# glennhickey/teHmm

Measured on AMD Instinct MI355X. Metric: genome positions/sec (Viterbi+posterior), 35 states x 10 tracks, higher is better.
Workload: dtype f64

## Files before the change

### tehmm_amd/csrc/tehmm_hip.hip

```cpp
#include <climits>
#include "tehmm_kernels.hip.h"
#include "tehmm_coop.hip.h"
#include "tehmm_lane.hip.h"
#include "tehmm_lane3.hip.h"
#include "tehmm_place.hip.h"
#include "tehmm_aux.hip.h"
#include "tehmm_fused.hip.h"
#include "tehmm_estep.hip.h"
#include "tehmm_wide_estep.hip.h"
#include "tehmm_wide.hip.h"
#include "tehmm_large.hip.h"
#include "tehmm_map.hip.h"
#include "tehmm_edist.hip.h"
#include "tehmm_segment.hip.h"
#include "tehmm_compare.hip.h"
#include "tehmm_tsd.hip.h"
#include "tehmm_masking.hip.h"
#include "tehmm_trackio.hip.h"
#include "tehmm_scaling.hip.h"

#include <algorithm>
#include <atomic>
#include <cmath>
#include <cstdio>
// ... 1146 lines not shown

template <int NT>
static void launch_vit_coop(tehmm_batch *b, const tehmm_model *m, const IntervalTab &iv,
                            const EmisTab &em, bool ratio, hipStream_t st) {
  constexpr int CPB = NT <= 44 ? 64 : 32;
  size_t lds = ((size_t)3 * CPB * (NT + 1) + 2 * (CPB + 1) * (NT + 2) + (size_t)m->lds_rows * NT) * sizeof(double);
  if (ratio) {
    allow_lds(k_vit_coop<NT, CPB, true>, lds);
    hipLaunchKernelGGL((k_vit_coop<NT, CPB, true>), dim3(b->n), dim3(256), lds, st, iv, em, m->N,
                       m->lt.p, m->ltT.p, m->pi.p, b->ratios.p, b->tb.p, b->last_state.p, b->vit_lp.p);
  } else {
    allow_lds(k_vit_coop<NT, CPB, false>, lds);
    hipLaunchKernelGGL((k_vit_coop<NT, CPB, false>), dim3(b->n), dim3(256), lds, st, iv, em, m->N,
                       m->lt.p, m->ltT.p, m->pi.p, (const double *)nullptr, b->tb.p, b->last_state.p,
                       b->vit_lp.p);
  }
}

template <int NT>
static void launch_fb_coop(tehmm_batch *b, const tehmm_model *m, const IntervalTab &iv,
                           const EmisTab &em_in, hipStream_t st) {
  constexpr int CPB = NT <= 44 ? 64 : 32;
  const EmisTab em = b->n > 256 ? without_lds_tables(em_in) : em_in;
  size_t lds = ((size_t)4 * CPB * (NT + 1) + 4 * CPB + 5 * NT + (size_t)em.lds_rows * NT) * sizeof(double);
  allow_lds(k_fb_coop<NT, CPB, false>, lds);
  hipLaunchKernelGGL((k_fb_coop<NT, CPB, false>), dim3(b->n), dim3(256), lds, st, iv, em, m->N, m->A.p,
                     m->lt.p, m->pi.p, (const double *)nullptr, b->post.p, b->beta.p, b->fwd_lp.p,
                     b->dead.p, (double *)nullptr, (int *)nullptr);
}

static int spec_chunk_size() {
  const char *s = std::getenv("TEHMM_SPEC_CHUNK");
  int cs = s ? std::atoi(s) : 512;
  if (cs <= 0) return 0;
  return std::max(64, (cs + 63) & ~63);
}

#define TEHMM_ESTEP_SMALL_DEFAULT 40

struct EvalKnobs {
  int spec_chunk;
  bool spec_chunk_set;
  int lane_sub;
  int lane_warmup;
  bool lane_probe;
  bool lane_vit;
  bool lane_p0;
  bool fused;
  bool device_place;
  bool soft_ties;
  int emis_split;
  int defer;
  int gain_window;
  bool rowindex_ref;
  bool wide;
  bool wide_cp;
  bool wide_vit;
  int wide_sub;
  int wide_vit_warmup;
  double wide_tol;
  bool wide_head;
  bool wide_poll;
  int estep_wide;
  bool estep_fused;
  int estep_small;
  int wide_estep_sq;
  bool wide_estep_serial;
};

static EvalKnobs read_eval_knobs() {
  auto num = [](const char *name, int unset) {
    const char *s = std::getenv(name);
    return s ? std::atoi(s) : unset;
  };
  EvalKnobs k;
  k.spec_chunk = spec_chunk_size();
  k.spec_chunk_set = std::getenv("TEHMM_SPEC_CHUNK") != nullptr;
  k.lane_sub = std::getenv("TEHMM_LANE_SUB") ? std::max(0, num("TEHMM_LANE_SUB", 0)) : -1;
  k.lane_warmup = std::getenv("TEHMM_LANE_WARMUP") ? std::max(1, num("TEHMM_LANE_WARMUP", 1)) : -1;
  k.lane_probe = num("TEHMM_LANE_PROBE", 1) != 0;
  k.lane_vit = num("TEHMM_LANE_VIT", 1) != 0;
  k.lane_p0 = num("TEHMM_LANE_P0", 1) != 0;
  k.fused = num("TEHMM_FUSED", 1) != 0;
  k.device_place = num("TEHMM_DEVICE_PLACE", 1) != 0;
  k.soft_ties = num("TEHMM_SOFT_TIES", 1) != 0;
  k.emis_split = std::getenv("TEHMM_EMIS_SPLIT") ? (num("TEHMM_EMIS_SPLIT", 0) != 0 ? 1 : 0) : -1;
  k.defer = num("TEHMM_DEFER", -1);
  k.gain_window = std::getenv("TEHMM_GAIN_WINDOW") ? std::max(0, num("TEHMM_GAIN_WINDOW", 0)) : -1;
  k.rowindex_ref = num("TEHMM_ROWINDEX_REF", 0) != 0;
  k.wide = num("TEHMM_WIDE", 1) != 0;
  k.wide_cp = num("TEHMM_WIDE_CP", 1) != 0;
  k.wide_vit = num("TEHMM_WIDE_VIT", 1) != 0;
  k.wide_sub = std::getenv("TEHMM_WIDE_SUB") ? std::max(32, (num("TEHMM_WIDE_SUB", 0) + 31) & ~31) : -1;
  k.wide_vit_warmup = std::max(0, num("TEHMM_WIDE_VIT_WARMUP", 32));
  k.wide_tol = 1e-8;
  if (const char *ts = std::getenv("TEHMM_WIDE_TOL")) k.wide_tol = std::min(1e-6, std::max(1e-13, std::atof(ts)));
  k.wide_head = num("TEHMM_WIDE_HEAD", 1) != 0;
  k.wide_poll = num("TEHMM_WIDE_POLL", 1) != 0;
  k.estep_wide = num("TEHMM_ESTEP_WIDE", 1);
  k.estep_fused = num("TEHMM_ESTEP_FUSED", 1) != 0;
  k.estep_small = num("TEHMM_ESTEP_SMALL", TEHMM_ESTEP_SMALL_DEFAULT);
  k.wide_estep_sq = num("TEHMM_WIDE_ESTEP_SQ", 0);
  k.wide_estep_serial = std::getenv("TEHMM_WIDE_ESTEP_SERIAL") != nullptr;
  return k;
}

static int spec_prepare(tehmm_batch *b, const tehmm_model *m, int CS) {
  SpecWork &sw = b->sw;
  if (sw.CS == CS && sw.N == m->N && sw.rows.p) return TEHMM_OK;
  sw.CS = CS;
  sw.N = m->N;
  sw.h_iv.clear();
  sw.h_t0.clear();
  sw.h_first.assign((size_t)b->n + 1, 0);
  for (int i = 0; i < b->n; ++i) {
    sw.h_first[i] = (int64_t)sw.h_iv.size();
    for (int64_t t0 = 0; t0 < b->h_len[i]; t0 += CS) {
      sw.h_iv.push_back(i);
      sw.h_t0.push_back(t0);
    }
  }
  sw.h_first[b->n] = (int64_t)sw.h_iv.size();
  sw.n_chunks = (int)sw.h_iv.size();
  const size_t nc = (size_t)std::max(1, sw.n_chunks);
  HIPCHK(sw.iv.upload(sw.h_iv.data(), sw.h_iv.size()));
  HIPCHK(sw.t0.upload(sw.h_t0.data(), sw.h_t0.size()));
  HIPCHK(sw.first.upload(sw.h_first.data(), sw.h_first.size()));
  HIPCHK(sw.e.alloc(nc));
  HIPCHK(sw.ok.alloc(nc));
  HIPCHK(sw.stats.alloc(16));
  HIPCHK(hipMemset(sw.stats.p, 0, 16 * sizeof(int)));
  HIPCHK(sw.scale.alloc(nc * (size_t)(CS / 32)));
  HIPCHK(sw.wstart.alloc(nc * (size_t)m->NP));
  HIPCHK(sw.gain.alloc(nc));
  HIPCHK(sw.wmin.alloc(nc));
  HIPCHK(sw.rows.alloc(nc * (size_t)(CS / TEHMM_VROW) * m->NP));
  HIPCHK(sw.ntie.alloc(nc));
  HIPCHK(sw.ties.alloc(nc * TEHMM_SPEC_MAXT));
  HIPCHK(sw.tierows.alloc(nc * TEHMM_SPEC_MAXT * (size_t)m->NP));
  HIPCHK(sw.segmin.alloc(nc * (TEHMM_SPEC_MAXT + 1)));
  HIPCHK(sw.offend.alloc(nc));
// ... 324 lines not shown

static int launch_vit_place(tehmm_batch *b, const tehmm_model *m, const IntervalTab &iv, int CS, int Wn, bool ratio,
                            hipStream_t st, int *n_work_max) {
  LaneWork &lw = b->lw;
  SpecWork &sw = b->sw;
  const LaneGeom lg = lane_geom(lw);
  hipLaunchKernelGGL(k_vit_place_chunks, dim3(std::max(1, b->n)), dim3(64), 0, st, iv, (const int64_t *)sw.first.p,
                     (const int64_t *)sw.t0.p, (const int64_t *)lw.ifirst.p, b->n, CS, lw.L, (const double *)lw.vgain.p,
                     (const double *)lw.slog32.p, Wn, (const int *)m->qok[ratio ? 1 : 0].p, kSpecMarginRel, kSpecCross ? 1 : 0, sw.e.p,
                     sw.gain.p);
  const int gb = (lw.n_groups + 255) / 256;
  hipLaunchKernelGGL(k_vit_place_count, dim3(std::max(1, gb)), dim3(256), 0, st, lg, (const int64_t *)sw.first.p,
                     (const int *)sw.e.p, CS, lw.place.p, lw.gclass.p);
  hipLaunchKernelGGL(k_vit_place_scan, dim3(1), dim3(64), 0, st, lw.place.p);
  hipLaunchKernelGGL(k_vit_place_fill, dim3(std::max(1, gb)), dim3(256), 0, st, lg, (const int64_t *)sw.first.p,
                     (const int *)sw.e.p, CS, lw.place.p, (const int *)lw.gclass.p, lw.wk_g.p, lw.wk_e.p, lw.wk_items.p);
  *n_work_max = 2 * lw.n_groups + TEHMM_PLACE_NE;
  return TEHMM_OK;
}

template <int NT>
static void launch_vit_stitch(tehmm_batch *b, const tehmm_model *m, const IntervalTab &iv, const VitChunks &vc,
                              hipStream_t st) {
  LaneWork &lw = b->lw;
  hipLaunchKernelGGL((k_vit_stitch<NT>), dim3((vc.n + 3) / 4), dim3(256), 0, st, iv, lane_geom(lw), vc,
                     lane_vit_items(lw), m->N, lw.soft_ties);
  hipLaunchKernelGGL((k_vit_links<NT>), dim3((vc.n + 3) / 4), dim3(256), 0, st, iv, lane_geom(lw), vc,
                     lane_vit_items(lw), m->N);
  hipLaunchKernelGGL(k_vit_runs, dim3(std::max(1, b->n)), dim3(64), 0, st, vc, b->n);
}

static LaneGeom lane_geom(const LaneWork &lw) {
  LaneGeom lg;
  lg.item_iv = lw.item_iv.p; lg.item_t0 = lw.item_t0.p; lg.ifirst = lw.ifirst.p;
  lg.n_items = lw.n_items; lg.n_groups = lw.n_groups; lg.L = lw.L;
  return lg;
}

template <int NT>
static void launch_emis_lane(tehmm_batch *b, const tehmm_model *m, const IntervalTab &iv, const EmisTab &em,
                             bool want_log, bool want_lin, bool want_f32, hipStream_t st) {
  LaneWork &lw = b->lw;
  const size_t lds = (size_t)em.lds_rows * NT * sizeof(double);
  allow_lds(k_emis_lane<NT>, lds);
  hipLaunchKernelGGL((k_emis_lane<NT>), dim3((lw.n_groups + 3) / 4), dim3(256), lds, st, iv, em, lane_geom(lw),
                     m->N, want_log ? lw.B.p : (double *)nullptr, want_lin ? lw.BH.p : (double *)nullptr, lw.MS.p,
                     want_f32 ? lw.B32.p : (float *)nullptr);
}

static bool emis_gain_split(int NT, int n_groups, int emis_split) {
  return NT >= 12 && (emis_split >= 0 ? emis_split != 0 : n_groups < 2048);
}

template <int NT>
static void launch_emis_gain_lane(tehmm_batch *b, const tehmm_model *m, const IntervalTab &iv, const EmisTab &em,
                                  int CS, int Wu, int Wn, bool ratio, int emis_split, hipStream_t st) {
  LaneWork &lw = b->lw;
  if constexpr (NT >= 12) {
    if (emis_gain_split(NT, lw.n_groups, emis_split)) {
      constexpr int NW = TEHMM_P2_NW, NU = 2;
      const size_t lds3 = Emis3Geom<NT, NW, NU>::lds_bytes(em.lds_rows);
      const dim3 grid3((lw.n_groups + NU - 1) / NU);
      if constexpr (NT <= TEHMM_RATIO_LANE_MAX) if (ratio) {
        allow_lds(k_emis_gain_lane3<NT, NW, NU, true>, lds3);
        hipLaunchKernelGGL((k_emis_gain_lane3<NT, NW, NU, true>), grid3, dim3(64 * NW * NU), lds3, st, iv, em, lane_geom(lw),
                           m->N, CS, Wu, (const float *)m->ltP.p, lw.B.p, lw.vgain.p, (const double *)b->ratios.p);
        return;
      }
      allow_lds(k_emis_gain_lane3<NT, NW, NU, false>, lds3);
      hipLaunchKernelGGL((k_emis_gain_lane3<NT, NW, NU, false>), grid3, dim3(64 * NW * NU), lds3, st, iv, em, lane_geom(lw),
                         m->N, CS, Wu, (const float *)m->ltP.p, lw.B.p, lw.vgain.p, (const double *)nullptr);
      return;
    }
  }
  const size_t lds = (size_t)em.lds_rows * NT * sizeof(double);
  if constexpr (NT <= TEHMM_RATIO_LANE_MAX) if (ratio) {
    allow_lds(k_emis_gain_lane<NT, true>, lds);
    hipLaunchKernelGGL((k_emis_gain_lane<NT, true>), dim3((lw.n_groups + 3) / 4), dim3(256), lds, st, iv, em,
                       lane_geom(lw), m->N, CS, Wu, 0, (const float *)m->ltP.p, lw.B.p, lw.vgain.p,
                       (const double *)b->ratios.p);
    return;
  }
  if (Wn > 0) {
    allow_lds(k_emis_gain_lane<NT, false, true>, lds);
    hipLaunchKernelGGL((k_emis_gain_lane<NT, false, true>), dim3((lw.n_groups + 3) / 4), dim3(256), lds, st, iv, em,
                       lane_geom(lw), m->N, CS, Wu, Wn, (const float *)m->ltP.p, lw.B.p, lw.vgain.p,
                       (const double *)nullptr);
    return;
  }
  allow_lds(k_emis_gain_lane<NT>, lds);
  hipLaunchKernelGGL((k_emis_gain_lane<NT>), dim3((lw.n_groups + 3) / 4), dim3(256), lds, st, iv, em, lane_geom(lw),
                     m->N, CS, Wu, 0, (const float *)m->ltP.p, lw.B.p, lw.vgain.p, (const double *)nullptr);
}

template <int NT>
static void launch_gain_lane(tehmm_batch *b, const tehmm_model *m, const IntervalTab &iv, int CS, int Wu,
                             hipStream_t st) {
  LaneWork &lw = b->lw;
  hipLaunchKernelGGL((k_vit_gain_lane<NT>), dim3((lw.n_groups + 3) / 4), dim3(256), 0, st, iv, lane_geom(lw), m->N,
                     CS, Wu, (const float *)m->ltP.p, (const float *)lw.B32.p, lw.vgain.p);
}

template <int NT>
static void launch_fb_lane(tehmm_batch *b, const tehmm_model *m, const IntervalTab &iv, const EmisTab &em_in,
                           const FbChunks &fc, int Wu, hipStream_t st, hipEvent_t ev_mid) {
  LaneWork &lw = b->lw;
  const LaneGeom lg = lane_geom(lw);
  const dim3 grid((lw.n_groups + 3) / 4);
  const dim3 gridc((fc.n + 255) / 256);
  const dim3 gridit((lw.n_items + 255) / 256);
  const dim3 gridi(std::max(1, b->n));
  const EmisTab em = b->n > 256 ? without_lds_tables(em_in) : em_in;
  size_t lds = ((size_t)2 * 64 * (NT + 1) + 2 * 64 + NT + (size_t)em.lds_rows * NT + 8) * sizeof(double);
  allow_lds(k_fb_fix<NT, 0, false, true>, lds);
  allow_lds(k_fb_fix<NT, 1, false, true>, lds);
  hipStream_t sS = b->sB;
  hipLaunchKernelGGL((k_fb_lane<NT, 0>), grid, dim3(256), 0, st, iv, lg, m->N, fc.CS, Wu, m->AG.p, lw.BH.p,
                     lw.MS.p, lw.AL.p, lw.pre_f.p, lw.end_f.p, lw.slog32.p);
  (void)hipEventRecord(b->evX[0], st);
  (void)hipStreamWaitEvent(sS, b->evX[0], 0);
  hipLaunchKernelGGL((k_fb_itemlinks<NT>), gridit, dim3(256), 0, sS, lg, m->N, lw.pre_f.p, lw.end_f.p, lw.pre_b.p,
                     lw.end_b.p, lw.dl_f.p, lw.lr_f.p, lw.dl_b.p, 1);
  hipLaunchKernelGGL((k_fb_stitch<NT>), gridc, dim3(256), 0, sS, iv, lg, fc, m->N, lw.slog32.p, lw.end_b.p,
                     lw.dl_f.p, lw.lr_f.p, lw.dl_b.p, lw.ok_f.p, lw.ok_b.p, 1);
  hipLaunchKernelGGL(k_fb_runs, gridi, dim3(64), 0, sS, iv, fc, (const int *)lw.ok_f.p, (const int *)lw.ok_b.p,
                     1);
  hipLaunchKernelGGL((k_fb_fix<NT, 0, false, true>), dim3(b->n), dim3(128), lds, sS, iv, em, fc, m->N, m->A.p,
                     m->lt.p, m->pi.p, (const double *)nullptr, lw.AL.p, b->fwd_lp.p, b->dead.p,
                     (double *)nullptr, (int *)nullptr, 1, b->sw.stats.p, lg, (const int *)lw.ok_f.p);
  (void)hipEventRecord(b->evX[1], sS);
  hipLaunchKernelGGL((k_fb_lane<NT, 1>), grid, dim3(256), 0, st, iv, lg, m->N, fc.CS, Wu, m->ATG.p, lw.BH.p,
                     lw.MS.p, lw.BE.p, lw.pre_b.p, lw.end_b.p, (double *)nullptr);
  hipLaunchKernelGGL((k_fb_itemlinks<NT>), gridit, dim3(256), 0, st, lg, m->N, lw.pre_f.p, lw.end_f.p, lw.pre_b.p,
// ... 738 lines not shown
                                 nullptr, b->tb.p, b->last_state.p, b->vit_lp.p, st);
    else
      launch_vit_large<uint8_t>(iv, em, lg, b->n, ratio, false, m->lt.p, m->pi.p, ratio ? b->ratios.p : nullptr,
                                nullptr, b->tb.p, b->last_state.p, b->vit_lp.p, st);
    (void)hipEventRecord(b->ev[1], st);
    const int rc = wide_ptr ? traceback_large<uint16_t>(iv, b->n, b->h_chunk0.data(), b->n_chunks, b->d_chunk_iv.p,
                                                        b->d_chunk0.p, m->N, m->NP, b->tb.p, b->G.p, b->bstate.p, b->Gg,
                                                        b->tstate, b->last_state.p, b->paths.p, st)
                            : traceback_large<uint8_t>(iv, b->n, b->h_chunk0.data(), b->n_chunks, b->d_chunk_iv.p,
                                                       b->d_chunk0.p, m->N, m->NP, b->tb.p, b->G.p, b->bstate.p, b->Gg,
                                                       b->tstate, b->last_state.p, b->paths.p, st);
    if (rc) return rc;
    (void)hipEventRecord(b->ev[2], st);
    add_stage(b, "k_vit_large", 0, 1);
    add_stage(b, "traceback", 1, 2);
  }
  if (postr) {
    add_stage(b, "k_fwd_large", 5, 6);
    add_stage(b, "k_bwd_large", 6, 7);
  }
  HIPCHK(hipGetLastError());
  if (vit) HIPCHK(hipStreamSynchronize(b->sV));
  if (postr) HIPCHK(hipStreamSynchronize(b->sP));
  stage_times(b);
  if (vit && viterbi_logprob)
    HIPCHK(hipMemcpy(viterbi_logprob, b->vit_lp.p, (size_t)b->n * sizeof(double), hipMemcpyDeviceToHost));
  if (postr) {
    b->h_fwd_lp.resize((size_t)b->n);
    HIPCHK(hipMemcpy(b->h_fwd_lp.data(), b->fwd_lp.p, (size_t)b->n * sizeof(double), hipMemcpyDeviceToHost));
    if (forward_logprob) std::memcpy(forward_logprob, b->h_fwd_lp.data(), (size_t)b->n * sizeof(double));
  }
  return TEHMM_OK;
}

constexpr int eV = 0, eP = 5;

struct EvalPlan {
  bool vit, postr;
  bool ratio;
  bool coop;
  int SPL;
  int CS;
  bool vspec;
  bool fspec;
  bool fused_fb;
  int LS;
  bool vlane;
  bool flane;
  bool glane;
  bool emis_gain;
  bool dev_place;
  int WuV;
  int gain_window;
  int defer_mode;
  bool defer_post;
  bool split_post;
  bool wide_defer;
};

static EvalPlan plan_eval(const tehmm_model *m, const tehmm_batch *b, int flags, const EvalKnobs &kn) {
  EvalPlan p{};
  p.vit = flags & TEHMM_EVAL_VITERBI;
  p.postr = flags & TEHMM_EVAL_POSTERIOR;
  p.ratio = (flags & TEHMM_EVAL_USE_RATIOS) && b->has_ratios;
  p.coop = m->N < 64;
  p.SPL = m->N <= 64 ? 1 : 2;
  p.CS = kn.spec_chunk;
  const bool spec_ok = p.coop && p.CS > 0 && m->NP <= 64 && b->total >= 2 * (int64_t)p.CS;
  p.vspec = p.vit && spec_ok && (!p.ratio || (ratio_lane_ok(m) && m->NP <= TEHMM_RATIO_LANE_MAX));
  p.fspec = p.postr && spec_ok;
  p.fused_fb = kn.fused && m->ptab.p != nullptr && m->K <= 78;
  p.LS = (p.vspec || p.fspec) ? lane_sub_size(p.CS, b->total, kn.lane_sub) : 0;
  return p;
}

static int plan_lanes(EvalPlan &p, const tehmm_model *m, tehmm_batch *b, const EvalKnobs &kn) {
  LaneWork &lw = b->lw;
  if (p.LS > 0 && !lw.AL.p && !lw.AL32.p && !lw.B.p && !lw.B32.p) {
    size_t free_b = 0, total_b = 0;
    HIPCHK(dev_mem_info(&free_b, &total_b));
    const double per = (double)b->total * m->NP * 8.0;
    const double fb_units = p.fspec ? (p.fused_fb ? 0.7 : 3.2) : 0.0, p0_units = (p.vspec && !p.fused_fb) ? 0.5 : 0.0;
    lw.no_vlane = per * (fb_units + p0_units + 1.0) > 0.85 * (double)free_b;
    if (per * (fb_units + p0_units) > 0.85 * (double)free_b) p.LS = 0;
  }
  bool want_vlane = kn.lane_vit;
  if (p.LS > 0 && want_vlane && !lw.no_vlane && !lw.B.p && (lw.AL.p || lw.AL32.p || lw.B32.p)) {
    size_t free_b = 0, total_b = 0;
    HIPCHK(dev_mem_info(&free_b, &total_b));
    if ((double)b->total * m->NP * 8.0 * 1.6 > 0.85 * (double)free_b) lw.no_vlane = true;
  }
  if (lw.no_vlane) want_vlane = false;
  if (p.ratio && p.vspec && !(p.LS > 0 && want_vlane && (p.fused_fb || !(p.fspec && p.LS > 0)))) {
    p.vspec = false;
    if (!p.fspec) p.LS = 0;
  }
  p.vlane = p.vspec && p.LS > 0 && want_vlane;
  p.flane = p.fspec && p.LS > 0;
  p.glane = p.vspec && p.LS > 0 && (p.vlane || kn.lane_p0);
  p.emis_gain = p.glane && !(p.flane && !p.fused_fb);
  p.dev_place = kn.device_place && p.vlane && p.emis_gain;
  p.WuV = std::min(p.LS, 32);
  int64_t longest = 0;
  for (int i = 0; i < b->n; ++i) longest = std::max<int64_t>(longest, b->h_len[(size_t)i]);
  const bool big = b->total >= (int64_t)25000000 && 4 * longest <= b->total;
  p.defer_mode = kn.defer >= 0 ? kn.defer : (big ? 3 : 1);
  p.defer_post = p.vit && p.postr && p.vspec && (p.defer_mode == 1 || p.defer_mode == 3);
  p.split_post = p.defer_post && p.defer_mode == 3 && p.flane && p.fused_fb && p.vlane;
  p.wide_defer = p.vit && p.postr && !p.vspec && !p.coop && p.defer_mode != 0;
  p.gain_window = 0;
  return TEHMM_OK;
}

static void plan_gain_window(EvalPlan &p, const tehmm_model *m, const tehmm_batch *b, const EvalKnobs &kn) {
  if (!(p.split_post && p.dev_place && p.emis_gain && !p.ratio && p.LS >= 128 && p.LS % 32 == 0)) return;
  if (emis_gain_split(m->NP, b->lw.n_groups, kn.emis_split)) return;
  const int wn = (kn.gain_window >= 0 ? kn.gain_window : p.LS / 4) / 32 * 32;
  if (wn > 0 && wn + p.WuV <= p.LS) p.gain_window = wn;
}

struct EvalCtx {
  tehmm_model *m;
  tehmm_batch *b;
  const EvalPlan &p;
  const EvalKnobs &kn;
  IntervalTab iv;
  EmisTab em, emg;
  VitChunks vc;
  int WuF;
  bool wide_cp = false;
  bool wide_vit = false;
  bool wide_pending = false;
};

static int eval_place_setup(EvalCtx &c) {
  tehmm_batch *b = c.b;
  LaneWork &lw = b->lw;
  SpecWork &sw = b->sw;
  hipStream_t st = b->sV;
  int rc = ensure_qtabs(c.m, c.p.ratio);
  if (rc) return rc;
  const size_t ng = (size_t)std::max(1, lw.n_groups);
  HIPCHK(lw.wk_g.ensure(2 * ng + TEHMM_PLACE_NE));
  HIPCHK(lw.wk_e.ensure(2 * ng + TEHMM_PLACE_NE));
  HIPCHK(lw.wk_items.ensure((ng + TEHMM_PLACE_NE) * 64));
  HIPCHK(lw.gclass.ensure(ng));
  HIPCHK(lw.place.ensure(1));
  HIPCHK(hipMemsetAsync(lw.place.p, 0, sizeof(PlaceCounts), st));
  HIPCHK(hipMemsetAsync(lw.wk_items.p, 0xff, (ng + TEHMM_PLACE_NE) * 64 * sizeof(int), st));
  HIPCHK(hipMemsetAsync(sw.ok.p, 0, (size_t)std::max(1, sw.n_chunks) * sizeof(int), st));
  HIPCHK(hipMemsetAsync(sw.stats.p, 0, 2 * sizeof(int), st));
  HIPCHK(hipMemsetAsync(lw.vbad.p, 0, ng * 64 * sizeof(int), st));
  HIPCHK(hipMemsetAsync(lw.vntie.p, 0, ng * 64 * sizeof(int), st));
  return vit_lane_upload_args(b, c.vc, st);
}

static int eval_emis_p0(EvalCtx &c) {
  tehmm_batch *b = c.b;
  const tehmm_model *m = c.m;
  const EvalPlan &p = c.p;
  LaneWork &lw = b->lw;
  SpecWork &sw = b->sw;
  std::vector<double> &gain = lw.hs_gain;
  hipStream_t st = b->sV;
  if (p.vlane || p.glane) {
    if (p.emis_gain) {
      nt_dispatch(m->NP, [&](auto nt) {
        launch_emis_gain_lane<nt>(b, m, c.iv, c.em, p.CS, p.WuV, p.gain_window, p.ratio, c.kn.emis_split, st);
      });
    } else {
      nt_dispatch(m->NP, [&](auto nt) {
        launch_emis_lane<nt>(b, m, c.iv, c.em, p.vlane, p.flane && !p.fused_fb, p.glane, st);
      });
    }
    (void)hipEventRecord(b->ev[eV + 4], st);
    if (p.flane) {
      if (!p.fused_fb) {
        (void)hipEventRecord(b->evX[0], st);
        (void)hipStreamWaitEvent(b->sP, b->evX[0], 0);
      }
      (void)hipEventRecord(b->ev[eP + 4], b->sP);
    }
  }
  if (p.vspec) {
    if (p.glane) {
      if (!p.emis_gain) nt_dispatch(m->NP, [&](auto nt) { launch_gain_lane<nt>(b, m, c.iv, p.CS, p.WuV, st); });
      if (!p.dev_place) {
        gain.resize((size_t)std::max(1, lw.n_groups) * 64);
        HIPCHK(hipMemcpyAsync(gain.data(), lw.vgain.p, gain.size() * sizeof(double), hipMemcpyDeviceToHost, st));
      }
    } else {
      nt_dispatch(m->NP, [&](auto nt) { launch_vit_spec<nt>(b, m, c.iv, c.emg, c.vc, false, st); });
      gain.resize((size_t)std::max(1, sw.n_chunks));
      HIPCHK(hipMemcpyAsync(gain.data(), sw.gain.p, gain.size() * sizeof(double), hipMemcpyDeviceToHost, st));
    }
  }
  return TEHMM_OK;
}

static void eval_emission(EvalCtx &c) {
  const EvalPlan &p = c.p;
  if (!(p.flane && !p.fused_fb && !p.vlane && !p.glane)) return;
  tehmm_batch *b = c.b;
  hipStream_t st = b->sP;
  nt_dispatch(c.m->NP, [&](auto nt) { launch_emis_lane<nt>(b, c.m, c.iv, c.em, false, true, false, st); });
  (void)hipEventRecord(b->ev[eP + 4], st);
}

static FbChunks fb_chunks(const SpecWork &sw, const LaneWork &lw, int CS) {
  FbChunks fc{};
  fc.iv = sw.iv.p; fc.t0 = sw.t0.p; fc.first = sw.first.p; fc.n = sw.n_chunks; fc.CS = CS;
  fc.scale = sw.scale.p; fc.wstart = sw.wstart.p;
  fc.link_f = lw.link_f.p; fc.glog_f = lw.glog_f.p; fc.link_b = lw.link_b.p; fc.runend_f = lw.runend_f.p;
  fc.pre_f = lw.cpre_f.p; fc.runstart_b = lw.runstart_b.p;
  return fc;
}

static int eval_posterior(EvalCtx &c, int half) {
  tehmm_batch *b = c.b;
  const tehmm_model *m = c.m;
  const EvalPlan &p = c.p;
// ... 330 lines not shown
      add("forward_pass", 10, eP + 3);
      add("backward_posterior_pass", p.split_post ? 11 : eP + 3, eP + 1);
    } else if (p.flane) {
      if (!p.vlane && !p.glane) add("emission_rows", eP, eP + 4);
      add("forward_backward_speculate", 10, eP + 3);
      add("forward_backward", eP + 3, eP + 1);
    } else if (p.fspec) {
      add("forward_backward_speculate", eP, eP + 3);
      add("forward_backward", eP + 3, eP + 1);
    } else {
      add(p.coop ? "forward_backward" : "forward", eP, eP + 1);
    }
    add(p.flane && p.fused_fb ? "backward_chain" : (p.coop ? "posterior_combine" : "backward_posterior"), eP + 1, eP + 2);
  }
}

static int add_chain_counters(tehmm_batch *b) {
  int st[4] = {0, 0, 0, 0};
  HIPCHK(hipMemcpy(st, b->sw.stats.p + 2, sizeof(st), hipMemcpyDeviceToHost));
  add_counter(b, "count:forward_exact_blocks", st[0]);
  add_counter(b, "count:forward_chunk_jumps", st[1]);
  add_counter(b, "count:backward_exact_blocks", st[2]);
  add_counter(b, "count:backward_chunk_jumps", st[3]);
  return TEHMM_OK;
}

static int eval_counters(const EvalCtx &c) {
  tehmm_batch *b = c.b;
  auto add = [&](const char *name, double v) { add_counter(b, name, v); };
  if (c.p.fspec)
    if (int rc = add_chain_counters(b)) return rc;
  if (c.wide_cp) add("count:wide_chunk_parallel_warmup", b->ww.wu_ok);
  if (c.wide_vit) {
    int st2[2] = {0, 0};
    HIPCHK(hipMemcpy(st2, b->sw.stats.p, sizeof(st2), hipMemcpyDeviceToHost));
    add("count:viterbi_exact_blocks", st2[0]);
    add("count:viterbi_chunk_jumps", st2[1]);
  }
  if (c.p.vspec) {
    int st[4] = {0, 0, 0, 0};
    HIPCHK(hipMemcpy(st, b->sw.stats.p, sizeof(st), hipMemcpyDeviceToHost));
#ifdef TEHMM_CHAIN_PROF
    {
      int pr[4];
      HIPCHK(hipMemcpy(pr, b->sw.stats.p + 8, sizeof(pr), hipMemcpyDeviceToHost));
      HIPCHK(hipMemset(b->sw.stats.p + 8, 0, sizeof(pr)));
      std::fprintf(stderr, "[chain prof] summed over intervals, ms: prologue %.2f steps %.2f barrier %.2f\n", pr[0] * 1e-4,
                   pr[1] * 1e-4, pr[2] * 1e-4);
    }
#endif
    add("count:viterbi_exact_blocks", st[0]);
    add("count:viterbi_chunk_jumps", st[1]);
    add("count:gain_window", c.p.gain_window);
  }
  return TEHMM_OK;
}

int tehmm_eval_batch(tehmm_model_t *m, tehmm_batch_t *b, int flags, double *viterbi_logprob,
                     double *forward_logprob) {
  if (!m || !b) return fail(TEHMM_ERR_ARG, "tehmm_eval_batch: NULL handle");
  if (m->K != b->K) return fail(TEHMM_ERR_ARG, "tehmm_eval_batch: model/batch track count differ");
  if (!(flags & (TEHMM_EVAL_VITERBI | TEHMM_EVAL_POSTERIOR)))
    return fail(TEHMM_ERR_ARG, "tehmm_eval_batch: nothing to do");
  b->map_valid = false;
  reset_timings(b);
  if (b->n == 0 || b->total == 0) return TEHMM_OK;
  if (m->large) return eval_large(m, b, flags, viterbi_logprob, forward_logprob);
#ifdef TEHMM_DEV_NT
  if (m->N < 64 && m->NP != TEHMM_DEV_NT)
    return fail(TEHMM_ERR_UNSUPPORTED, "development build: fused kernels exist for one padded state count only");
#endif
  int rc = ensure_workspace(b, m, flags);
  if (rc) return rc;
  const EvalKnobs kn = read_eval_knobs();
  b->lw.rix_ref = kn.rowindex_ref;
  EvalPlan p = plan_eval(m, b, flags, kn);
  if (p.vspec || p.fspec) {
    rc = spec_prepare(b, m, p.CS);
    if (rc) return rc;
  }
  rc = plan_lanes(p, m, b, kn);
  if (rc) return rc;
  EvalCtx c{m, b, p, kn};
  fill_tabs(m, b, c.iv, c.em, false);
  c.emg = without_lds_tables(c.em);
  c.WuF = std::min(std::max(p.LS, 1), 64);
  if (p.vit) (void)hipEventRecord(b->ev[eV], b->sV);
  if (p.vlane || p.flane || p.glane) {
    rc = lane_prepare(b, m, p.CS, p.LS, p.flane, p.vlane, p.glane, p.fused_fb, !p.emis_gain);
    if (rc) return rc;
    plan_gain_window(p, m, b, kn);
  }
  if (p.flane) {
    rc = fb_warmup(b, m, p.LS, c.iv, c.emg, kn, &c.WuF);
    if (rc) return rc;
  }
  if (p.postr) (void)hipEventRecord(b->ev[eP], b->sP);
  if (p.vspec) {
    const SpecWork &sw = b->sw;
    VitChunks &vc = c.vc;
    vc.iv = sw.iv.p; vc.t0 = sw.t0.p; vc.first = sw.first.p; vc.n = sw.n_chunks; vc.CS = p.CS;
    vc.e = sw.e.p; vc.gain = sw.gain.p; vc.ok = sw.ok.p; vc.wmin = sw.wmin.p; vc.rows = sw.rows.p;
    vc.ntie = sw.ntie.p; vc.ties = sw.ties.p; vc.tierows = sw.tierows.p; vc.segmin = sw.segmin.p;
    vc.offend = sw.offend.p; vc.clink = sw.clink.p; vc.clk = sw.clk.p;
    vc.rtarget = sw.rtarget.p; vc.rsel = sw.rsel.p; vc.racc = sw.racc.p; vc.rmn = sw.rmn.p;
    vc.tsoft = sw.tsoft.p; vc.tpar = sw.tpar.p;
  }
  if (p.dev_place) {
    rc = eval_place_setup(c);
    if (rc) return rc;
  }
  if (p.split_post) {
    FusedOrder fo_unused;
    bool built = false;
    nt_dispatch(m->NP, [&](auto nt) { rc = fused_prepare<nt>(b, m, c.iv, c.WuF, b->sP, fo_unused, &built); });
    if (rc) return rc;
    if (built) {
      (void)hipEventRecord(b->evX[0], b->sP);
      (void)hipStreamWaitEvent(b->sV, b->evX[0], 0);
    }
  }
  rc = eval_emis_p0(c);
  if (rc) return rc;
  if (p.postr && p.defer_post) eval_emission(c);
  if (p.split_post) {
    rc = eval_posterior(c, 1);
    if (rc) return rc;
  } else if (p.postr && p.defer_post && p.flane && p.fused_fb) {
    FusedOrder fo_unused;
    nt_dispatch(m->NP, [&](auto nt) { rc = fused_prepare<nt>(b, m, c.iv, c.WuF, b->sP, fo_unused); });
    if (rc) return rc;
  }
  if (p.postr && !p.defer_post) {
    eval_emission(c);
    if (!p.wide_defer) {
      rc = eval_posterior(c, 0);
      if (rc) return rc;
    }
  }
  if (p.vit) {
    rc = eval_viterbi(c);
    if (rc) return rc;
  }
  rc = eval_finish_wide(c);
// ... 627 lines not shown
```

### tehmm_amd/csrc/tehmm_lane.hip.h

```cpp
#pragma once
#include "tehmm_spec.hip.h"

namespace tehmm {

typedef __attribute__((address_space(4))) const double const_f64;
#define TEHMM_TG(f, o, NT) ((((o) >> 2) * (NT) + (f)) * 4 + ((o) & 3))



template <int NT>
__global__ __launch_bounds__(256) void k_emis_lane(IntervalTab iv, EmisTab em, LaneGeom lg, int N,
                                                   double *B, double *BH, double *MS, float *B32) {
  extern __shared__ double emis_ltab[];
  stage_emis_table(em, emis_ltab, NT);
  __syncthreads();
  const int lane = threadIdx.x & 63;
  const int g = blockIdx.x * 4 + (threadIdx.x >> 6);
  if (g >= lg.n_groups) return;
  const int64_t item = (int64_t)g * 64 + lane;
  const bool valid = item < lg.n_items;
  const int id = valid ? lg.item_iv[item] : 0;
  const int64_t t0 = valid ? lg.item_t0[item] : 0;
  const int64_t T = iv.len[id], p0 = iv.pos0[id];
  const int len = valid ? (int)min((int64_t)lg.L, T - t0) : 0;
  const int maxlen = wave_max_i32(len);
  const double qnan = __longlong_as_double(0x7ff8000000000000LL);
  for (int s = 0; s < maxlen; ++s) {
    const bool act = s < len;
    const int64_t gpos = p0 + t0 + (act ? s : 0);
    double x[NT];
    emis_rows<NT>(em, emis_ltab, gpos, x);
    double m = x[0];
#pragma unroll
    for (int j = 1; j < NT; ++j) m = fmax(m, j < N ? x[j] : -INFINITY);
    const bool good = m > -1e20;
    if (act) {
      const int64_t o = ((((int64_t)g * lg.L + s) * NT) << 6) + lane;
      if (B) {
#pragma unroll
        for (int j = 0; j < NT; ++j) B[o + ((int64_t)j << 6)] = good ? x[j] : qnan;
      }
      if (B32) {
#pragma unroll
        for (int j = 0; j < NT; ++j) B32[o + ((int64_t)j << 6)] = good ? (float)x[j] : (float)qnan;
      }
      if (BH) {
#pragma unroll
        for (int j = 0; j < NT; ++j)
          BH[o + ((int64_t)j << 6)] = good ? (j < N ? exp_nonpos(x[j] - m) : 0.0) : qnan;
        MS[(((int64_t)g * lg.L + s) << 6) + lane] = m;
      }
    }
  }
}
// ... 875 lines not shown
                                                       const float *__restrict__ B32, double *gain) {
  const int lane = threadIdx.x & 63;
  const int g = blockIdx.x * 4 + (threadIdx.x >> 6);
  if (g >= lg.n_groups) return;
  const int L = lg.L;
  const int64_t item = (int64_t)g * 64 + lane;
  const bool valid = item < lg.n_items;
  const int id = valid ? lg.item_iv[item] : 0;
  const int64_t t0 = valid ? lg.item_t0[item] : 0;
  const int64_t T = iv.len[id];
  const int64_t ct0 = (t0 / CS) * CS;
  const bool run = valid && ct0 > 0 && ct0 + CS <= T;
  if (!__any(run)) return;
  const int64_t nb = run ? item - 1 : item;
  lane_f2 W[NT / 2];
#pragma unroll
  for (int j = 0; j < NT / 2; ++j)
    W[j] = (lane_f2){2 * j < N ? 0.f : -INFINITY, 2 * j + 1 < N ? 0.f : -INFINITY};
  bool bad = false;
  auto vec_max = [&]() {
    float mx = -INFINITY;
#pragma unroll
    for (int j = 0; j < NT / 2; ++j) mx = fmaxf(mx, fmaxf(W[j].x, W[j].y));
    return mx;
  };
  float g0 = 0.f;
  for (int s = -Wu; s < L; ++s) {
    if (s == 0) g0 = vec_max();
    const float *bp = B32 + (s < 0 ? lane_row(lg, NT, nb, L + s) : lane_row(lg, NT, item, s));
    float b[NT];
#pragma unroll
    for (int j = 0; j < NT; ++j) b[j] = bp[(int64_t)j << 6];
    bad = bad | (b[0] != b[0]);
    int z = 0;
    asm volatile("" : "+s"(z));
    const_f2 *tp = (const_f2 *)(size_t)tabf + z;
    lane_f2 x[NT / 2];
#pragma unroll
    for (int op = 0; op < NT / 2; ++op) {
      lane_f2 acc = (lane_f2){W[0].x, W[0].x} + tp[op * NT];
#pragma unroll
      for (int f = 1; f < NT; ++f) {
        const float wf = (f & 1) ? W[f >> 1].y : W[f >> 1].x;
        acc = __builtin_elementwise_max(acc, (lane_f2){wf, wf} + tp[op * NT + f]);
      }
      x[op] = acc;
    }
#pragma unroll
    for (int j = 0; j < NT / 2; ++j) W[j] = x[j] + (lane_f2){b[2 * j], b[2 * j + 1]};
  }
  if (run) gain[item] = bad ? __longlong_as_double(0x7ff8000000000000LL) : (double)vec_max() - (double)g0;
}

template <int NT, bool RATIO = false, bool WIN = false>
#ifndef TEHMM_EMIS_WAVES
#define TEHMM_EMIS_WAVES 2
#endif
__global__ __launch_bounds__(256) __attribute__((amdgpu_waves_per_eu(TEHMM_EMIS_WAVES, TEHMM_EMIS_WAVES))) void k_emis_gain_lane(IntervalTab iv, EmisTab em, LaneGeom lg, int N, int CS, int Wu, int Wn,
                                                        const float *__restrict__ tabf, double *B, double *gain,
                                                        const double *__restrict__ ratios = nullptr) {
  extern __shared__ double emis_ltab[];
  stage_emis_table(em, emis_ltab, NT);
  __syncthreads();
  const int lane = threadIdx.x & 63;
  const int g = blockIdx.x * 4 + (threadIdx.x >> 6);
  if (g >= lg.n_groups) return;
  const int L = lg.L;
  const int64_t item = (int64_t)g * 64 + lane;
  const bool valid = item < lg.n_items;
  const int id = valid ? lg.item_iv[item] : 0;
  const int64_t t0 = valid ? lg.item_t0[item] : 0;
  const int64_t T = iv.len[id], p0 = iv.pos0[id];
  const int len = valid ? (int)min((int64_t)L, T - t0) : 0;
  const int maxlen = wave_max_i32(len);
  const int64_t ct0 = (t0 / CS) * CS;
  const bool run = valid && ct0 > 0 && ct0 + CS <= T;
  const int s_first = WIN ? 0 : (__any(run) ? -Wu : 0);
  const int s_p0 = WIN ? L - Wn - Wu : s_first, s_g0 = WIN ? L - Wn : 0;
  const double qnan = __longlong_as_double(0x7ff8000000000000LL);
  lane_f2 W[NT / 2];
#pragma unroll
  for (int j = 0; j < NT / 2; ++j)
    W[j] = (lane_f2){2 * j < N ? 0.f : -INFINITY, 2 * j + 1 < N ? 0.f : -INFINITY};
  bool bad = false;
  auto vec_max = [&]() {
    float mx = -INFINITY;
#pragma unroll
    for (int j = 0; j < NT / 2; ++j) mx = fmaxf(mx, fmaxf(W[j].x, W[j].y));
    return mx;
  };
  float g0 = 0.f;
  for (int s = s_first; s < maxlen; ++s) {
    const bool act = s >= 0 ? s < len : run;
    const int64_t gpos = p0 + t0 + (act ? s : 0);
    double x[NT];
    emis_rows<NT>(em, emis_ltab, gpos, x);
    double m = x[0];
#pragma unroll
    for (int j = 1; j < NT; ++j) m = fmax(m, j < N ? x[j] : -INFINITY);
    const bool good = m > -1e20;
    if (B && s >= 0 && act) {
      const int64_t o = ((((int64_t)g * lg.L + s) * NT) << 6) + lane;
#pragma unroll
      for (int j = 0; j < NT; ++j) B[o + ((int64_t)j << 6)] = good ? x[j] : qnan;
    }
    bad = bad | (act && !good);
    if (WIN && s < s_p0) continue;
    if (s == s_g0) g0 = vec_max();
    int z = 0;
    asm volatile("" : "+s"(z));
    const_f2 *tp = (const_f2 *)(size_t)tabf + z;
    lane_f2 xn[NT / 2];
    float rf = 1.f, rm1 = 0.f;
    if (RATIO) {
      rf = (float)ratios[gpos];
      rm1 = rf > 1.f ? rf - 1.f : 0.f;
    }
#pragma unroll
    for (int op = 0; op < NT / 2; ++op) {
      lane_f2 acc = (lane_f2){W[0].x, W[0].x} + tp[op * NT];
      if (RATIO) {
        const lane_f2 ltd = tp[NT * NT / 2 + op];
        acc = acc + ltd * (lane_f2){rf - rm1, rf - rm1};
        if (op == 0) acc.x -= ((const float *)(size_t)tabf)[z + NT * NT + NT];
      }
#pragma unroll
      for (int f = 1; f < NT; ++f) {
        const float wf = (f & 1) ? W[f >> 1].y : W[f >> 1].x;
        acc = __builtin_elementwise_max(acc, (lane_f2){wf, wf} + tp[op * NT + f]);
      }
      xn[op] = acc;
    }
#pragma unroll
    for (int j = 0; j < NT / 2; ++j) {
      W[j] = xn[j] + (lane_f2){(float)x[2 * j], (float)x[2 * j + 1]};
      if (RATIO) W[j] = W[j] + tp[NT * NT / 2 + j] * (lane_f2){rm1, rm1};
    }
  }
  if (run) gain[item] = (bad || len < L) ? qnan : (double)vec_max() - (double)g0;
}

}
```

Before: 1.636 billion.

## Add fast emission-row path with LDS-staged observation prefetch in emis-gain lane kernel

```diff
diff --git a/tehmm_amd/csrc/tehmm_emis_fast.hip.h b/tehmm_amd/csrc/tehmm_emis_fast.hip.h
--- /dev/null
+++ b/tehmm_amd/csrc/tehmm_emis_fast.hip.h
@@ -0,0 +1,139 @@
+#pragma once
+#include "tehmm_coop.hip.h"
+
+namespace tehmm {
+
+#define TEHMM_EFAST_PB 4
+#define TEHMM_EFAST_WORDS (TEHMM_EFAST_PB * 3 + 2)
+#define TEHMM_EFAST_WAVE_BYTES (TEHMM_EFAST_WORDS * 256)
+#define TEHMM_EFAST_NT_MAX 36
+
+typedef unsigned int efast_u4 __attribute__((ext_vector_type(4)));
+typedef __attribute__((address_space(3))) unsigned int efast_lds_u32;
+
+struct ObsWindow {
+  const uint32_t *src;
+  unsigned stage;
+  int KPW, s0, lo, hi;
+  efast_u4 r[TEHMM_EFAST_PB * 3 / 4];
+
+  __device__ __forceinline__ void request(int blk) {
+    const int sb = s0 + blk * TEHMM_EFAST_PB;
+    const efast_u4 *p = (const efast_u4 *)(src + (int64_t)((sb >= lo && sb < hi) ? sb : 0) * KPW);
+#pragma unroll
+    for (int c = 0; c < TEHMM_EFAST_PB * 3 / 4; ++c)
+      if (c < TEHMM_EFAST_PB / 4 * KPW) r[c] = p[c];
+  }
+  __device__ __forceinline__ void commit() {
+    efast_lds_u32 *d = (efast_lds_u32 *)(size_t)stage;
+#pragma unroll
+    for (int c = 0; c < TEHMM_EFAST_PB * 3 / 4; ++c)
+      if (c < TEHMM_EFAST_PB / 4 * KPW) {
+        d[(4 * c + 0) * 64] = r[c].x;
+        d[(4 * c + 1) * 64] = r[c].y;
+        d[(4 * c + 2) * 64] = r[c].z;
+        d[(4 * c + 3) * 64] = r[c].w;
+      }
+  }
+  __device__ __forceinline__ void words(int rel, unsigned &w0, unsigned &w1, unsigned &w2) const {
+    const efast_lds_u32 *d = (const efast_lds_u32 *)(size_t)(stage + (unsigned)(rel * KPW) * 256u);
+    w0 = d[0];
+    w1 = d[64];
+    w2 = d[128];
+  }
+};
+
+template <int NT>
+struct EmisFastRows {
+  static constexpr int H = NT / 4;
+  static constexpr unsigned ROWB = NT * 8;
+  const char *tab;
+  int meta_cnt;
+  unsigned meta_base;
+  unsigned zero_lds, zero_glb;
+  int K, n_lds;
+  unsigned w0, w1, w2;
+
+  __device__ __forceinline__ void init(const EmisTab &em, const double *ltab, int lane) {
+    const unsigned la = (unsigned)(size_t)(__attribute__((address_space(3))) const double *)ltab;
+    const bool tr = lane < em.K;
+    const int lb = tr ? em.ldsbase[lane] : -1;
+    meta_cnt = tr ? em.rowcnt[lane] : 0;
+    meta_base = lb >= 0 ? la + (unsigned)lb * ROWB : (unsigned)(tr ? em.rowbase[lane] : 0) * ROWB;
+    n_lds = __popcll(__ballot(lb >= 0));
+    K = em.K;
+    tab = (const char *)em.tab;
+    zero_lds = la + (unsigned)em.lds_zero * ROWB;
+    zero_glb = (unsigned)em.zero_row * ROWB;
+  }
+  __device__ __forceinline__ unsigned row_of(int k, unsigned zero) {
+    const unsigned sym = w0 & 0xffu;
+    w0 = __builtin_amdgcn_alignbit(w1, w0, 8);
+    w1 = __builtin_amdgcn_alignbit(w2, w1, 8);
+    w2 >>= 8;
+    const unsigned cnt = (unsigned)__builtin_amdgcn_readlane(meta_cnt, k);
+    const unsigned base = (unsigned)__builtin_amdgcn_readlane((int)meta_base, k);
+    return sym < cnt ? base + sym * ROWB : zero;
+  }
+  template <int HALF>
+  static __device__ __forceinline__ void load_lds(unsigned a, d2v (&buf)[H]) {
+    lds_cd2 *p = (lds_cd2 *)(size_t)a;
+#pragma unroll
+    for (int i = 0; i < H; ++i) buf[i] = p[HALF * H + i];
+  }
+  template <int HALF>
+  __device__ __forceinline__ void load_glb(unsigned off, d2v (&buf)[H]) const {
+    const d2v *p = (const d2v *)(tab + off);
+#pragma unroll
+    for (int i = 0; i < H; ++i) buf[i] = p[HALF * H + i];
+  }
+  template <int HALF>
+  static __device__ __forceinline__ void add(double (&x)[NT], const d2v (&buf)[H]) {
+#pragma unroll
+    for (int i = 0; i < H; ++i) {
+      x[2 * (HALF * H + i)] += buf[i].x;
+      x[2 * (HALF * H + i) + 1] += buf[i].y;
+    }
+  }
+  __device__ __forceinline__ void rows(double (&x)[NT]) {
+#pragma unroll
+    for (int j = 0; j < NT; ++j) x[j] = 0.0;
+    d2v a[H], b[H];
+    if (n_lds > 0) {
+      unsigned ra = row_of(0, zero_lds);
+      asm volatile("v_mov_b32 %0, %1" : "=v"(ra) : "v"(ra));
+      load_lds<0>(ra, a);
+#pragma unroll 1
+      for (int k = 1; k < n_lds; ++k) {
+        load_lds<1>(ra, b);
+        ra = row_of(k, zero_lds);
+        asm volatile("v_mov_b32 %0, %1" : "=v"(ra) : "v"(ra));
+        add<0>(x, a);
+        load_lds<0>(ra, a);
+        add<1>(x, b);
+      }
+      load_lds<1>(ra, b);
+      add<0>(x, a);
+    }
+    if (n_lds < K) {
+      unsigned ro = row_of(n_lds, zero_glb);
+      load_glb<0>(ro, a);
+      if (n_lds > 0) add<1>(x, b);
+#pragma unroll 1
+      for (int k = n_lds + 1; k < K; ++k) {
+        load_glb<1>(ro, b);
+        ro = row_of(k, zero_glb);
+        add<0>(x, a);
+        load_glb<0>(ro, a);
+        add<1>(x, b);
+      }
+      load_glb<1>(ro, b);
+      add<0>(x, a);
+      add<1>(x, b);
+    } else {
+      add<1>(x, b);
+    }
+  }
+};
+
+}
diff --git a/tehmm_amd/csrc/tehmm_hip.hip b/tehmm_amd/csrc/tehmm_hip.hip
--- a/tehmm_amd/csrc/tehmm_hip.hip
+++ b/tehmm_amd/csrc/tehmm_hip.hip
@@ -1222,6 +1222,7 @@
   int emis_split;
   int defer;
   int gain_window;
+  bool emis_fast;
   bool rowindex_ref;
   bool wide;
   bool wide_cp;
@@ -1257,6 +1258,7 @@
   k.emis_split = std::getenv("TEHMM_EMIS_SPLIT") ? (num("TEHMM_EMIS_SPLIT", 0) != 0 ? 1 : 0) : -1;
   k.defer = num("TEHMM_DEFER", -1);
   k.gain_window = std::getenv("TEHMM_GAIN_WINDOW") ? std::max(0, num("TEHMM_GAIN_WINDOW", 0)) : -1;
+  k.emis_fast = num("TEHMM_EMIS_FAST", 1) != 0;
   k.rowindex_ref = num("TEHMM_ROWINDEX_REF", 0) != 0;
   k.wide = num("TEHMM_WIDE", 1) != 0;
   k.wide_cp = num("TEHMM_WIDE_CP", 1) != 0;
@@ -1687,9 +1689,21 @@
   return NT >= 12 && (emis_split >= 0 ? emis_split != 0 : n_groups < 2048);
 }
 
+static bool emis_fast_ok(const tehmm_model *m, const EmisTab &em, int Wu, bool ratio) {
+  if (ratio || em.ratios || em.normalize != 1.0 || em.K > 12 || em.KPW > 3) return false;
+  if (m->NP > TEHMM_EFAST_NT_MAX || m->N < m->NP - 3 || Wu % TEHMM_EFAST_PB != 0) return false;
+  if (((int64_t)em.zero_row + 1) * m->NP * 8 >= ((int64_t)1 << 31)) return false;
+  bool glb = false;
+  for (int k = 0; k < em.K; ++k) {
+    if (em.ldsbase[k] < 0) glb = true;
+    else if (glb) return false;
+  }
+  return true;
+}
+
 template <int NT>
 static void launch_emis_gain_lane(tehmm_batch *b, const tehmm_model *m, const IntervalTab &iv, const EmisTab &em,
-                                  int CS, int Wu, int Wn, bool ratio, int emis_split, hipStream_t st) {
+                                  int CS, int Wu, int Wn, bool ratio, int emis_split, bool fast, hipStream_t st) {
   LaneWork &lw = b->lw;
   if constexpr (NT >= 12) {
     if (emis_gain_split(NT, lw.n_groups, emis_split)) {
@@ -1714,6 +1728,21 @@
     hipLaunchKernelGGL((k_emis_gain_lane<NT, true>), dim3((lw.n_groups + 3) / 4), dim3(256), lds, st, iv, em,
                        lane_geom(lw), m->N, CS, Wu, 0, (const float *)m->ltP.p, lw.B.p, lw.vgain.p,
                        (const double *)b->ratios.p);
+    return;
+  }
+  if constexpr (NT <= TEHMM_EFAST_NT_MAX) if (fast) {
+    const size_t ldsf = lds + 4 * (size_t)TEHMM_EFAST_WAVE_BYTES;
+    if (Wn > 0) {
+      allow_lds(k_emis_gain_lane<NT, false, true, true>, ldsf);
+      hipLaunchKernelGGL((k_emis_gain_lane<NT, false, true, true>), dim3((lw.n_groups + 3) / 4), dim3(256), ldsf, st, iv, em,
+                         lane_geom(lw), m->N, CS, Wu, Wn, (const float *)m->ltP.p, lw.B.p, lw.vgain.p,
+                         (const double *)nullptr);
+    } else {
+      allow_lds(k_emis_gain_lane<NT, false, false, true>, ldsf);
+      hipLaunchKernelGGL((k_emis_gain_lane<NT, false, false, true>), dim3((lw.n_groups + 3) / 4), dim3(256), ldsf, st, iv, em,
+                         lane_geom(lw), m->N, CS, Wu, 0, (const float *)m->ltP.p, lw.B.p, lw.vgain.p,
+                         (const double *)nullptr);
+    }
     return;
   }
   if (Wn > 0) {
@@ -2558,6 +2587,7 @@
   bool dev_place;
   int WuV;
   int gain_window;
+  bool emis_fast;
   int defer_mode;
   bool defer_post;
   bool split_post;
@@ -2623,6 +2653,11 @@
   if (emis_gain_split(m->NP, b->lw.n_groups, kn.emis_split)) return;
   const int wn = (kn.gain_window >= 0 ? kn.gain_window : p.LS / 4) / 32 * 32;
   if (wn > 0 && wn + p.WuV <= p.LS) p.gain_window = wn;
+}
+
+static void plan_emis_fast(EvalPlan &p, const tehmm_model *m, const tehmm_batch *b, const EmisTab &em, const EvalKnobs &kn) {
+  p.emis_fast = kn.emis_fast && (p.vlane || p.glane) && p.emis_gain &&
+                !emis_gain_split(m->NP, b->lw.n_groups, kn.emis_split) && emis_fast_ok(m, em, p.WuV, p.ratio);
 }
 
 struct EvalCtx {
@@ -2672,7 +2707,7 @@
   if (p.vlane || p.glane) {
     if (p.emis_gain) {
       nt_dispatch(m->NP, [&](auto nt) {
-        launch_emis_gain_lane<nt>(b, m, c.iv, c.em, p.CS, p.WuV, p.gain_window, p.ratio, c.kn.emis_split, st);
+        launch_emis_gain_lane<nt>(b, m, c.iv, c.em, p.CS, p.WuV, p.gain_window, p.ratio, c.kn.emis_split, p.emis_fast, st);
       });
     } else {
       nt_dispatch(m->NP, [&](auto nt) {
@@ -3109,6 +3144,7 @@
     add("count:viterbi_exact_blocks", st[0]);
     add("count:viterbi_chunk_jumps", st[1]);
     add("count:gain_window", c.p.gain_window);
+    add("count:emis_fast", c.p.emis_fast ? 1 : 0);
   }
   return TEHMM_OK;
 }
@@ -3147,6 +3183,7 @@
     rc = lane_prepare(b, m, p.CS, p.LS, p.flane, p.vlane, p.glane, p.fused_fb, !p.emis_gain);
     if (rc) return rc;
     plan_gain_window(p, m, b, kn);
+    plan_emis_fast(p, m, b, c.em, kn);
   }
   if (p.flane) {
     rc = fb_warmup(b, m, p.LS, c.iv, c.emg, kn, &c.WuF);
diff --git a/tehmm_amd/csrc/tehmm_lane.hip.h b/tehmm_amd/csrc/tehmm_lane.hip.h
--- a/tehmm_amd/csrc/tehmm_lane.hip.h
+++ b/tehmm_amd/csrc/tehmm_lane.hip.h
@@ -1,5 +1,6 @@
 #pragma once
 #include "tehmm_spec.hip.h"
+#include "tehmm_emis_fast.hip.h"
 
 namespace tehmm {
 
@@ -981,7 +982,7 @@
   if (run) gain[item] = bad ? __longlong_as_double(0x7ff8000000000000LL) : (double)vec_max() - (double)g0;
 }
 
-template <int NT, bool RATIO = false, bool WIN = false>
+template <int NT, bool RATIO = false, bool WIN = false, bool FAST = false>
 #ifndef TEHMM_EMIS_WAVES
 #define TEHMM_EMIS_WAVES 2
 #endif
@@ -1019,19 +1020,62 @@
     return mx;
   };
   float g0 = 0.f;
+  ObsWindow ow;
+  EmisFastRows<NT> fr;
+  if (FAST) {
+    fr.init(em, emis_ltab, lane);
+    ow.src = em.obs32 + (p0 + t0) * em.KPW;
+    ow.stage = (unsigned)(size_t)(__attribute__((address_space(3))) const double *)emis_ltab +
+               (unsigned)(em.lds_rows * NT * 8) + (threadIdx.x >> 6) * TEHMM_EFAST_WAVE_BYTES + lane * 4;
+    ow.KPW = em.KPW;
+    ow.s0 = s_first;
+    ow.lo = run ? s_first : 0;
+    ow.hi = len;
+    ow.request(0);
+    ow.commit();
+    ow.request(1);
+  }
   for (int s = s_first; s < maxlen; ++s) {
     const bool act = s >= 0 ? s < len : run;
     const int64_t gpos = p0 + t0 + (act ? s : 0);
     double x[NT];
-    emis_rows<NT>(em, emis_ltab, gpos, x);
-    double m = x[0];
-#pragma unroll
-    for (int j = 1; j < NT; ++j) m = fmax(m, j < N ? x[j] : -INFINITY);
-    const bool good = m > -1e20;
-    if (B && s >= 0 && act) {
-      const int64_t o = ((((int64_t)g * lg.L + s) * NT) << 6) + lane;
-#pragma unroll
-      for (int j = 0; j < NT; ++j) B[o + ((int64_t)j << 6)] = good ? x[j] : qnan;
+    bool good;
+    if (FAST) {
+      const int rel = (s - s_first) & (TEHMM_EFAST_PB - 1);
+      ow.words(rel, fr.w0, fr.w1, fr.w2);
+      fr.rows(x);
+      if (rel == TEHMM_EFAST_PB - 1) {
+        ow.commit();
+        ow.request((s - s_first) / TEHMM_EFAST_PB + 2);
+      }
+      double m = x[0];
+#pragma unroll
+      for (int j = 1; j < NT; ++j) m = fmax(m, (j < NT - 3 || j < N) ? x[j] : -INFINITY);
+      good = m > -1e20;
+      if (__any(!good)) {
+        if (B && s >= 0 && act) {
+          const int64_t o = ((((int64_t)g * lg.L + s) * NT) << 6) + lane;
+          double q = qnan;
+          asm volatile("" : "+v"(q));
+#pragma unroll
+          for (int j = 0; j < NT; ++j) B[o + ((int64_t)j << 6)] = good ? x[j] : q;
+        }
+      } else if (B && s >= 0 && act) {
+        const int64_t o = ((((int64_t)g * lg.L + s) * NT) << 6) + lane;
+#pragma unroll
+        for (int j = 0; j < NT; ++j) __builtin_nontemporal_store(x[j], &B[o + ((int64_t)j << 6)]);
+      }
+    } else {
+      emis_rows<NT>(em, emis_ltab, gpos, x);
+      double m = x[0];
+#pragma unroll
+      for (int j = 1; j < NT; ++j) m = fmax(m, j < N ? x[j] : -INFINITY);
+      good = m > -1e20;
+      if (B && s >= 0 && act) {
+        const int64_t o = ((((int64_t)g * lg.L + s) * NT) << 6) + lane;
+#pragma unroll
+        for (int j = 0; j < NT; ++j) B[o + ((int64_t)j << 6)] = good ? x[j] : qnan;
+      }
     }
     bad = bad | (act && !good);
     if (WIN && s < s_p0) continue;
```

Result: faster. 1.677 billion, median of 6 (+2.5%).
